# Wangshihu12/Voxel-SLAM

Hardware: AMD Instinct MI355X
Metric: local-BA iterations/sec (200k pts, W=10) (higher is better)
Workload: dtype f64

## Files before the change

### voxel-slam_amd/csrc/vba_kernels_factor.hpp

```cpp
#pragma once
#include <hip/hip_runtime.h>
#include "vba_eig3.hpp"

namespace vba {

struct FactorView {
  double *cl;
  double *fix;
  double *coe;
  double *eigval;
  double *eigvec;
  double *pcr;
  unsigned int *occ;
  int *tiles;
  int vs;
  int W;
};

__host__ __device__ inline int mask_bucket(unsigned int m, int nb) {
  constexpr int C[11][11] = {{1, 0, 0, 0, 0, 0, 0, 0, 0, 0, 0}, {1, 1, 0, 0, 0, 0, 0, 0, 0, 0, 0}, {1, 2, 1, 0, 0, 0, 0, 0, 0, 0, 0}, {1, 3, 3, 1, 0, 0, 0, 0, 0, 0, 0},
                             {1, 4, 6, 4, 1, 0, 0, 0, 0, 0, 0}, {1, 5, 10, 10, 5, 1, 0, 0, 0, 0, 0}, {1, 6, 15, 20, 15, 6, 1, 0, 0, 0, 0},
                             {1, 7, 21, 35, 35, 21, 7, 1, 0, 0, 0}, {1, 8, 28, 56, 70, 56, 28, 8, 1, 0, 0}, {1, 9, 36, 84, 126, 126, 84, 36, 9, 1, 0},
                             {1, 10, 45, 120, 210, 252, 210, 120, 45, 10, 1}};
  int p = 0;
// ... 344 lines not shown
  if (lane == 63) partial[blockIdx.x] = r;
  if (STAMPS && lane == 0 && blockIdx.x < 2048) {
    st3 = clock64();
    long long *o = stamps + (size_t)blockIdx.x * 4;
    o[0] = st0; o[1] = st1; o[2] = st2; o[3] = st3;
  }
}

__global__ __launch_bounds__(256) void k_reduce_partials(const double *__restrict__ partial, int nb, int nout, double *__restrict__ out,
                                                        const int *__restrict__ gate) {
  __shared__ double s[256];
  const int gate_v = gate ? *gate : 1;
  const int j = threadIdx.x & 15, q = threadIdx.x >> 4;
  const int o = blockIdx.x * 16 + j, oc = o < nout ? o : nout - 1;
  double pv[16];
#pragma unroll
  for (int k = 0; k < 16; k++) { const int b = q + 16 * k; pv[k] = partial[(size_t)(b < nb ? b : 0) * nout + oc]; }
#pragma unroll
  for (int k = 0; k < 16; k++) asm volatile("" : "+v"(pv[k]));
  if (gate_v == 0) return;
  double acc = 0.0;
  if (o < nout) {
#pragma unroll
    for (int k = 0; k < 16; k++) acc += (q + 16 * k < nb) ? pv[k] : 0.0;
    for (int b = q + 256; b < nb; b += 16) acc += partial[(size_t)b * nout + o];
  }
  s[threadIdx.x] = acc;
  __syncthreads();
  if (q == 0 && o < nout) {
    double t = 0.0;
#pragma unroll
    for (int k = 0; k < 16; k++) t += s[16 * k + j];
    out[o] = t;
  }
}

__global__ __launch_bounds__(256) void k_sum_scalar(const double *__restrict__ partial, int nb, double *__restrict__ out,
                                                   const int *__restrict__ gate) {
  __shared__ double s[4];
  if (gate && *gate == 0) return;
  double acc = 0.0;
  for (int b = threadIdx.x; b < nb; b += 256) acc += partial[b];
  acc = wave_sum(acc);
  if ((threadIdx.x & 63) == 0) s[threadIdx.x >> 6] = acc;
  __syncthreads();
  if (threadIdx.x == 0) out[0] = (s[0] + s[1]) + (s[2] + s[3]);
}

typedef double v4f64 __attribute__((ext_vector_type(4)));

constexpr int hess2_tv(int W) {
  return W == 2 ? 128 : W == 3 ? 80 : W == 4 ? 64 : W == 5 ? 48 : W == 6 ? 40 : (W == 7 || W == 8) ? 32 : (W == 9 || W == 10) ? 24 : 16;
}
constexpr int gcd_i(int a, int b) { return b == 0 ? a : gcd_i(b, a % b); }

__device__ __forceinline__ double rcp_f64(double x) {
  double y = __builtin_amdgcn_rcp(x);
  y = y * (2.0 - x * y);
  y = y * (2.0 - x * y);
  return y;
}

template <int W>
struct HessCfg2 {
  static constexpr int TV = hess2_tv(W);
  static constexpr int NT = 256;
  static constexpr int NC = 6 * W;
  static constexpr int NT16 = (NC + 15) / 16;
  static constexpr int NCP = 16 * NT16;
  static constexpr int GS = ((NCP % 32 == 16) ? NCP : NCP + 16) + 1;
  static constexpr int NK = 3 * TV;
  static constexpr int NWV = NT / 64;
  static constexpr int NU = NT16 * (NT16 + 1) / 2;
  static constexpr int KS = NWV / gcd_i(NU, NWV);
  static constexpr int UPW = NU * KS / NWV;
  static constexpr int KSTEPS = NK / 4 / KS;
  static constexpr int NOUT = NC * NC + NC + 1;
  static constexpr int EB = NU * 256;
  static constexpr int GB = EB + 21 * W;
  static constexpr int RB = GB + 6 * W;
  static constexpr int NOUT2 = RB + 1;
  static constexpr int NG8 = NT / 8;
  static_assert(TV * W <= NT && TV % 8 == 0 && (NK / 4) % KS == 0 && (NU * KS) % NWV == 0, "tile shape");
  static constexpr bool PRESCALE = ((size_t)2 * NK * GS + NK + W * 12 + 8) * sizeof(double) <= (size_t)150 * 1024;
  static constexpr size_t LDS_MAIN = (size_t)NK * GS * (PRESCALE ? 2 : 1) + NK + W * 12 + 8;
  static constexpr size_t LDS_EPI = (size_t)(KS > 1 ? NU * 256 : 0) + (size_t)28 * NG8 + 8;
  static constexpr size_t LDS_BYTES = (LDS_MAIN > LDS_EPI ? LDS_MAIN : LDS_EPI) * sizeof(double);
};

struct SlotLoad {
  double n, c[9], coe, l0, l1, l2, NN, vs0, vs1, vs2, U[9];
  bool valid;
};

template <int W>
__device__ __forceinline__ void slot_load(const FactorView &f, int v, int fi, int end, unsigned int occm, SlotLoad &q) {
  const size_t vs = (size_t)f.vs, fs = (size_t)W * vs;
  q.valid = v < end;
  if (q.valid) {
    const double *cp = f.cl + (size_t)fi * vs + v;
    const bool on = (occm >> fi) & 1u;
    q.n = on ? cp[9 * fs] : 0.0;
#pragma unroll
    for (int k = 0; k < 9; k++) q.c[k] = on ? cp[(size_t)k * fs] : 0.0;
    q.coe = f.coe[v];
    q.l0 = f.eigval[v]; q.l1 = f.eigval[vs + v]; q.l2 = f.eigval[2 * vs + v];
    q.NN = f.pcr[9 * vs + v]; q.vs0 = f.pcr[6 * vs + v]; q.vs1 = f.pcr[7 * vs + v]; q.vs2 = f.pcr[8 * vs + v];
#pragma unroll
    for (int k = 0; k < 9; k++) q.U[k] = f.eigvec[(size_t)k * vs + v];
  }
}

__device__ __forceinline__ void slot_terms(const SlotLoad &q, const double *R, bool first, double *g1, double *g2, double *hh, double &ck1, double &ck2, double &ck3,
                                           double *Err, double *Ert, double *Ett, double *gj, double &rres) {
if (q.valid) {
  const double coe = q.coe, l0 = q.l0, NN = q.NN;
  const double inn = rcp_f64(NN);
  const double c1 = 2.0 * rcp_f64(l0 - q.l1), c2 = 2.0 * rcp_f64(l0 - q.l2);
  ck1 = coe * c1; ck2 = coe * c2; ck3 = coe * (-2.0 * inn * inn);
  if (first) rres += coe * l0;
  const double n = q.n;
  if (n != 0.0) {
    const double pxx = q.c[0], pxy = q.c[1], pxz = q.c[2], pyy = q.c[3], pyz = q.c[4], pzz = q.c[5];
    const double vx = q.c[6], vy = q.c[7], vz = q.c[8];
    const double u00 = q.U[0], u01 = q.U[1], u02 = q.U[2], u10 = q.U[3], u11 = q.U[4], u12 = q.U[5], u20 = q.U[6], u21 = q.U[7], u22 = q.U[8];
    const double bx = q.vs0 * inn, by = q.vs1 * inn, bz = q.vs2 * inn;
    
    const double k0 = u00, k1 = u10, k2 = u20;
    const double a00 = R[0] * k0 + R[3] * k1 + R[6] * k2, a01 = R[1] * k0 + R[4] * k1 + R[7] * k2, a02 = R[2] * k0 + R[5] * k1 + R[8] * k2;
    const double a10 = R[0] * u01 + R[3] * u11 + R[6] * u21, a11 = R[1] * u01 + R[4] * u11 + R[7] * u21, a12 = R[2] * u01 + R[5] * u11 + R[8] * u21;
    const double a20 = R[0] * u02 + R[3] * u12 + R[6] * u22, a21 = R[1] * u02 + R[4] * u12 + R[7] * u22, a22 = R[2] * u02 + R[5] * u12 + R[8] * u22;
    const double tx = R[9] - bx, ty = R[10] - by, tz = R[11] - bz;
    const double s0 = k0 * tx + k1 * ty + k2 * tz, s1 = u01 * tx + u11 * ty + u21 * tz, s2 = u02 * tx + u12 * ty + u22 * tz;
    const double pa00 = pxx * a00 + pxy * a01 + pxz * a02, pa01 = pxy * a00 + pyy * a01 + pyz * a02, pa02 = pxz * a00 + pyz * a01 + pzz * a02;
    const double pa10 = pxx * a10 + pxy * a11 + pxz * a12, pa11 = pxy * a10 + pyy * a11 + pyz * a12, pa12 = pxz * a10 + pyz * a11 + pzz * a12;
    const double pa20 = pxx * a20 + pxy * a21 + pxz * a22, pa21 = pxy * a20 + pyy * a21 + pyz * a22, pa22 = pxz * a20 + pyz * a21 + pzz * a22;
    const double wx = pa00 + s0 * vx, wy = pa01 + s0 * vy, wz = pa02 + s0 * vz;
    const double c2x = R[0] * vx + R[1] * vy + R[2] * vz + n * tx;
    const double c2y = R[3] * vx + R[4] * vy + R[5] * vz + n * ty;
    const double c2z = R[6] * vx + R[7] * vy + R[8] * vz + n * tz;
    const double qx = vy * a02 - vz * a01, qy = vz * a00 - vx * a02, qz = vx * a01 - vy * a00;
    const double d0 = c2x * k0 + c2y * k1 + c2z * k2;
    const double d1 = c2x * u01 + c2y * u11 + c2z * u21;
    const double d2 = c2x * u02 + c2y * u12 + c2z * u22;
    const double j0 = 2.0 * (wy * a02 - wz * a01) * inn, j1 = 2.0 * (wz * a00 - wx * a02) * inn, j2 = 2.0 * (wx * a01 - wy * a00) * inn;
    const double j3 = 2.0 * d0 * k0 * inn, j4 = 2.0 * d0 * k1 * inn, j5 = 2.0 * d0 * k2 * inn;
    gj[0] += coe * j0; gj[1] += coe * j1; gj[2] += coe * j2; gj[3] += coe * j3; gj[4] += coe * j4; gj[5] += coe * j5;
    {
      const double bx1 = pa10 + s1 * vx, by1 = pa11 + s1 * vy, bz1 = pa12 + s1 * vz;
      g1[0] = (-(a01 * bz1 - a02 * by1) + (wy * a12 - wz * a11)) * inn;
      g1[1] = (-(a02 * bx1 - a00 * bz1) + (wz * a10 - wx * a12)) * inn;
      g1[2] = (-(a00 * by1 - a01 * bx1) + (wx * a11 - wy * a10)) * inn;
      g1[3] = (k0 * d1 + d0 * u01) * inn; g1[4] = (k1 * d1 + d0 * u11) * inn; g1[5] = (k2 * d1 + d0 * u21) * inn;
      const double bx2 = pa20 + s2 * vx, by2 = pa21 + s2 * vy, bz2 = pa22 + s2 * vz;
      g2[0] = (-(a01 * bz2 - a02 * by2) + (wy * a22 - wz * a21)) * inn;
      g2[1] = (-(a02 * bx2 - a00 * bz2) + (wz * a20 - wx * a22)) * inn;
      g2[2] = (-(a00 * by2 - a01 * bx2) + (wx * a21 - wy * a20)) * inn;
      g2[3] = (k0 * d2 + d0 * u02) * inn; g2[4] = (k1 * d2 + d0 * u12) * inn; g2[5] = (k2 * d2 + d0 * u22) * inn;
    }
    hh[0] = qx; hh[1] = qy; hh[2] = qz; hh[3] = n * k0; hh[4] = n * k1; hh[5] = n * k2;
    const double wa = wx * a00 + wy * a01 + wz * a02;
    const double t00 = a01 * pxz - a02 * pxy, t10 = a02 * pxx - a00 * pxz, t20 = a00 * pxy - a01 * pxx;
    const double t01 = a01 * pyz - a02 * pyy, t11 = a02 * pxy - a00 * pyz, t21 = a00 * pyy - a01 * pxy;
    const double t02 = a01 * pzz - a02 * pyz, t12 = a02 * pxz - a00 * pzz, t22 = a00 * pyz - a01 * pxz;
    const double S00 = t01 * a02 - t02 * a01, S01 = -t00 * a02 + t02 * a00, S02 = t00 * a01 - t01 * a00;
    const double S11 = -t10 * a02 + t12 * a00, S12 = t10 * a01 - t11 * a00;
    const double S22 = t20 * a01 - t21 * a00;
    const double e2 = 2.0 * inn * coe;
    Err[0] += e2 * (a00 * wx - wa - S00);
    Err[1] += e2 * (0.5 * (a00 * wy + wx * a01) - S01);
    Err[2] += e2 * (0.5 * (a00 * wz + wx * a02) - S02);
    Err[3] += e2 * (a01 * wy - wa - S11);
    Err[4] += e2 * (0.5 * (a01 * wz + wy * a02) - S12);
    Err[5] += e2 * (a02 * wz - wa - S22);
    Ert[0] += e2 * qx * k0; Ert[1] += e2 * qx * k1; Ert[2] += e2 * qx * k2;
    Ert[3] += e2 * qy * k0; Ert[4] += e2 * qy * k1; Ert[5] += e2 * qy * k2;
    Ert[6] += e2 * qz * k0; Ert[7] += e2 * qz * k1; Ert[8] += e2 * qz * k2;
    const double e3 = e2 * n;
    Ett[0] += e3 * k0 * k0; Ett[1] += e3 * k0 * k1; Ett[2] += e3 * k0 * k2; Ett[3] += e3 * k1 * k1; Ett[4] += e3 * k1 * k2; Ett[5] += e3 * k2 * k2;
  }
}
}

struct LmDev;
__device__ int lm_prev_stop(const LmDev *s);
__device__ double lm_r1(const LmDev *s);
__device__ const double *lm_xt(const LmDev *s);
__device__ void lm_update_apply(LmDev *s, double r2, int W);
__device__ __forceinline__ double lm_sum_partials(const double *__restrict__ r2_dev, int nb, int lane) {
  double pv[8];
#pragma unroll
  for (int k = 0; k < 8; k++) { const int b = lane + 64 * k; pv[k] = r2_dev[(nb > 0 && b < nb) ? b : 0]; }
  double acc = 0.0;
#pragma unroll
  for (int k = 0; k < 8; k++) acc += (lane + 64 * k < nb) ? pv[k] : 0.0;
  for (int b = lane + 512; b < nb; b += 64) acc += r2_dev[b];
  for (int m = 32; m >= 1; m >>= 1) acc += __shfl_xor(acc, m, 64);
  return acc;
}

struct LiDev;
struct LiJob { const LmDev *lm; LiDev *dev; const double *imu; double *himu, *gimu; };
__device__ void li_imu_body(const LmDev *s, LiDev *li, const double *imu, double *himu, double *gimu, double *lds);

template <int W>
__global__ __launch_bounds__(HessCfg2<W>::NT) void k_hessian2(FactorView f, const double *__restrict__ poses, int head, int end,
                                                             int ntiles, double *__restrict__ partial, const int *__restrict__ gate,
                                                             long long *__restrict__ stamps, LmDev *lm, const double *__restrict__ k4_partial, int k4_nb,
                                                             int nwg, LiJob li) {
  using C = HessCfg2<W>;
  extern __shared__ __attribute__((aligned(16))) double lds[];
  if (li.dev && blockIdx.x == 0) {
    li_imu_body(li.lm, li.dev, li.imu, li.himu, li.gimu, lds);
    return;
  }
  const int bid = (int)blockIdx.x - (li.dev ? 1 : 0);
  const int tile0 = (int)(((long long)bid * ntiles) / nwg), tile1 = (int)(((long long)(bid + 1) * ntiles) / nwg);
  const int my_vl = threadIdx.x % HessCfg2<W>::TV, my_fi = threadIdx.x / HessCfg2<W>::TV;
  unsigned int occ_nx = 0;
  if (my_fi < W && tile0 < tile1) { const int v0 = head + tile0 * HessCfg2<W>::TV + my_vl; occ_nx = f.occ[v0 < end ? v0 : end - 1]; }
  __shared__ int lm_dec[2];
  int gate_v = (gate && !lm) ? *gate : 1;
  double lm_r2 = 0.0;
  if (lm) {
    if (threadIdx.x < 64) {
      lm_r2 = lm_sum_partials(k4_partial, k4_nb, threadIdx.x);
      if (threadIdx.x == 0) {
        const double r1 = lm_r1(lm);
        const int stop = lm_prev_stop(lm);
        const bool accept = (r1 - lm_r2) > 0, nstop = fabs((r1 - lm_r2) / r1) < 1e-6;
        lm_dec[0] = (!stop && accept && !nstop) ? 1 : 0;
        lm_dec[1] = stop;
      }
    }
    poses = lm_xt(lm);
  }
#define VBA_STAMP(i) do { if (stamps && threadIdx.x == 0) stamps[(size_t)bid * 16 + (i)] = wall_clock64(); } while (0)
  VBA_STAMP(0);
  double *G = lds;
  double *GA = C::PRESCALE ? G + (size_t)C::NK * C::GS : G;
  double *cK = GA + (size_t)C::NK * C::GS;
  double *sp = cK + C::NK;
  const int tid = threadIdx.x, lane = tid & 63, wv = tid >> 6;

  for (int t = tid; t < W * 12; t += C::NT) sp[t] = poses[t];
  constexpr int PADC = C::GS - C::NC;
  if constexpr (PADC > 0)
    for (int t = tid; t < C::NK * PADC; t += C::NT) { G[(size_t)(t / PADC) * C::GS + C::NC + t % PADC] = 0.0; if (C::PRESCALE) GA[(size_t)(t / PADC) * C::GS + C::NC + t % PADC] = 0.0; }

  const int vl = tid % C::TV, fi = tid / C::TV;
  const bool slot_thread = fi < W;
  v4f64 acc[C::UPW];
#pragma unroll
  for (int t = 0; t < C::UPW; t++) acc[t] = (v4f64){0.0, 0.0, 0.0, 0.0};
  double Err[6] = {0, 0, 0, 0, 0, 0}, Ert[9] = {0, 0, 0, 0, 0, 0, 0, 0, 0}, Ett[6] = {0, 0, 0, 0, 0, 0};
  double gj[6] = {0, 0, 0, 0, 0, 0};
  double rres = 0.0;

  SlotLoad nx;
  nx.valid = false;
  if (slot_thread && tile0 < tile1) slot_load<W>(f, head + tile0 * C::TV + vl, fi, end, occ_nx, nx);
  if (slot_thread && tile0 + 1 < tile1) { const int v1 = head + (tile0 + 1) * C::TV + vl; occ_nx = f.occ[v1 < end ? v1 : end - 1]; }
  asm volatile("" : "+v"(nx.n));
  if (gate_v == 0) return;
  __syncthreads();
  if (lm) {
    const int run = lm_dec[0], was_stopped = lm_dec[1];
    if (bid == 0 && threadIdx.x < 64 && !was_stopped) lm_update_apply(lm, lm_r2, W);
    if (!run) return;
  }
  VBA_STAMP(1);
  int stamp_i = 2;

  for (int tile = tile0; tile < tile1; tile++) {
    if (slot_thread) {
      const SlotLoad q = nx;
      double g1[6] = {0, 0, 0, 0, 0, 0}, g2[6] = {0, 0, 0, 0, 0, 0}, hh[6] = {0, 0, 0, 0, 0, 0};
      double ck1 = 0.0, ck2 = 0.0, ck3 = 0.0;
      slot_terms(q, sp + 12 * fi, fi == 0, g1, g2, hh, ck1, ck2, ck3, Err, Ert, Ett, gj, rres);
      double *g = G + (size_t)(3 * vl) * C::GS + 6 * fi;
#pragma unroll
      for (int d = 0; d < 6; d++) { g[d] = g1[d]; g[C::GS + d] = g2[d]; g[2 * C::GS + d] = hh[d]; }
      if (C::PRESCALE) {
        double *ga = GA + (size_t)(3 * vl) * C::GS + 6 * fi;
#pragma unroll
        for (int d = 0; d < 6; d++) { ga[d] = g1[d] * ck1; ga[C::GS + d] = g2[d] * ck2; ga[2 * C::GS + d] = hh[d] * ck3; }
      }
      if (fi == 0) { cK[3 * vl] = ck1; cK[3 * vl + 1] = ck2; cK[3 * vl + 2] = ck3; }
      const int nt = tile + 1;
      nx.valid = false;
      if (nt < tile1) {
        slot_load<W>(f, head + nt * C::TV + vl, fi, end, occ_nx, nx);
        if (nt + 1 < tile1) { const int v2 = head + (nt + 1) * C::TV + vl; occ_nx = f.occ[v2 < end ? v2 : end - 1]; }
      }
    }
    __syncthreads();
    if (stamp_i < 12) { VBA_STAMP(stamp_i); stamp_i++; }
    {
      const int kr = lane >> 4, cl = lane & 15;
      const double *gap[C::UPW], *gbp[C::UPW], *ckp[C::UPW];
#pragma unroll
      for (int t = 0; t < C::UPW; t++) {
        const int unit = wv * C::UPW + t;
        const int u = unit % C::NU, ksp = unit / C::NU;
        int p = u, ta = 0;
        while (p >= C::NT16 - ta) { p -= C::NT16 - ta; ta++; }
        const int tb = ta + p;
        const int kb = ksp * C::KSTEPS * 4;
        gap[t] = GA + (size_t)(kb + kr) * C::GS + 16 * ta + cl;
        gbp[t] = G + (size_t)(kb + kr) * C::GS + 16 * tb + cl;
        ckp[t] = cK + kb + kr;
      }
      double ar[C::UPW], cr[C::UPW], br[C::UPW];
#pragma unroll
      for (int t = 0; t < C::UPW; t++) { ar[t] = gap[t][0]; cr[t] = C::PRESCALE ? 1.0 : ckp[t][0]; br[t] = gbp[t][0]; }
#pragma unroll
      for (int ks = 0; ks < C::KSTEPS; ks++) {
        double av[C::UPW], bv[C::UPW];
#pragma unroll
        for (int t = 0; t < C::UPW; t++) { av[t] = C::PRESCALE ? ar[t] : ar[t] * cr[t]; bv[t] = br[t]; }
        if (ks + 1 < C::KSTEPS) {
          const int k = 4 * (ks + 1);
#pragma unroll
          for (int t = 0; t < C::UPW; t++) { ar[t] = gap[t][(size_t)k * C::GS]; if (!C::PRESCALE) cr[t] = ckp[t][k]; br[t] = gbp[t][(size_t)k * C::GS]; }
        }
        __builtin_amdgcn_sched_barrier(0);
#pragma unroll
        for (int t = 0; t < C::UPW; t++) acc[t] = __builtin_amdgcn_mfma_f64_16x16x4f64(av[t], bv[t], acc[t], 0, 0, 0);
        __builtin_amdgcn_sched_barrier(0);
      }
    }
    __syncthreads();
    if (stamp_i < 12) { VBA_STAMP(stamp_i); stamp_i++; }
  }
  VBA_STAMP(12);

  double *out = partial + (size_t)bid * C::NOUT2;
  double *Tb = lds;
  double *Eb = Tb + (C::KS > 1 ? C::NU * 256 : 0);
  if (C::KS > 1) {
#pragma unroll
    for (int t = 0; t < C::UPW; t++) {
      const int unit = wv * C::UPW + t;
      if (unit / C::NU != 0) {
        const int u = unit % C::NU;
#pragma unroll
        for (int r = 0; r < 4; r++) {
          if (unit / C::NU == 1) Tb[u * 256 + r * 64 + lane] = acc[t][r];
        }
      }
    }
    for (int ksp = 2; ksp < C::KS; ksp++) {
      __syncthreads();
#pragma unroll
      for (int t = 0; t < C::UPW; t++) {
        const int unit = wv * C::UPW + t;
        if (unit / C::NU == ksp) {
          const int u = unit % C::NU;
#pragma unroll
          for (int r = 0; r < 4; r++) Tb[u * 256 + r * 64 + lane] += acc[t][r];
        }
      }
    }
  }
#pragma unroll
  for (int k = 0; k < 6; k++) { Err[k] = group8_sum(Err[k]); Ett[k] = group8_sum(Ett[k]); gj[k] = group8_sum(gj[k]); }
#pragma unroll
  for (int k = 0; k < 9; k++) Ert[k] = group8_sum(Ert[k]);
  rres = group8_sum(rres);
  if ((tid & 7) == 0) {
    const int g8 = tid >> 3;
#pragma unroll
    for (int k = 0; k < 6; k++) { Eb[(size_t)k * C::NG8 + g8] = Err[k]; Eb[(size_t)(15 + k) * C::NG8 + g8] = Ett[k]; Eb[(size_t)(21 + k) * C::NG8 + g8] = gj[k]; }
#pragma unroll
    for (int k = 0; k < 9; k++) Eb[(size_t)(6 + k) * C::NG8 + g8] = Ert[k];
    Eb[(size_t)27 * C::NG8 + g8] = rres;
  }
  __syncthreads();
  VBA_STAMP(13);
#pragma unroll
  for (int t = 0; t < C::UPW; t++) {
    const int unit = wv * C::UPW + t;
    if (unit / C::NU == 0) {
      const int u = unit % C::NU;
#pragma unroll
      for (int r = 0; r < 4; r++) {
        double val = acc[t][r];
        if (C::KS > 1) val += Tb[u * 256 + r * 64 + lane];
        out[u * 256 + r * 64 + lane] = val;
      }
    }
  }
  for (int t = tid; t < 28 * W; t += C::NT) {
    const int k = t % 28, fr = t / 28;
    double sum = 0.0;
#pragma unroll
    for (int g = 0; g < C::TV / 8; g++) sum += Eb[(size_t)k * C::NG8 + fr * (C::TV / 8) + g];
    if (k < 21) out[C::EB + 21 * fr + k] = sum;
    else if (k < 27) out[C::GB + 6 * fr + (k - 21)] = sum;
    else if (fr == 0) out[C::RB] = sum;
  }
  VBA_STAMP(14);
#undef VBA_STAMP
}

template <int W>
__device__ __forceinline__ double tl_fetch(const double *__restrict__ red, int row, int col) {
  using C = HessCfg2<W>;
  if (row > col) { const int t = row; row = col; col = t; }
  const int ta = row >> 4, tb = col >> 4;
  const int u = ta * C::NT16 - ta * (ta - 1) / 2 + (tb - ta);
  const int rt = row & 15, ct = col & 15;
  double val = red[u * 256 + (rt >> 2) * 64 + (rt & 3) * 16 + ct];
  const int fr = row / 6;
  if (col / 6 == fr) {
    const int a = row - 6 * fr, b = col - 6 * fr;
    int idx;
    if (b < 3) idx = a * 3 - a * (a - 1) / 2 + (b - a);
    else if (a < 3) idx = 6 + 3 * a + (b - 3);
    else { const int a2 = a - 3, b2 = b - 3; idx = 15 + a2 * 3 - a2 * (a2 - 1) / 2 + (b2 - a2); }
    val += red[C::EB + 21 * fr + idx];
  }
  return val;
}

template <int W>
__global__ void k_tiles_to_full(const double *__restrict__ red, double *__restrict__ full) {
  using C = HessCfg2<W>;
  for (int t = blockIdx.x * blockDim.x + threadIdx.x; t < C::NOUT; t += gridDim.x * blockDim.x) {
    if (t < C::NC * C::NC) full[t] = tl_fetch<W>(red, t / C::NC, t % C::NC);
    else if (t < C::NC * C::NC + C::NC) full[t] = red[C::GB + (t - C::NC * C::NC)];
    else full[t] = red[C::RB];
  }
}

}
```

### voxel-slam_amd/csrc/voxelba.hip

```cpp
#include "../../include/voxelba.h"

#define VBA_MAX_WIN_DEV VBA_MAX_WIN
#include "vba_kernels_factor.hpp"
#include "vba_kernels_h3.hpp"
#include "vba_kernels_map.hpp"
#include "vba_kernels_lm.hpp"
#include "vba_kernels_li.hpp"
#include "vba_kernels_scan.hpp"
#include "vba_kernels_gba.hpp"
#include "vba_kernels_big.hpp"
#include "vba_kernels_kd.hpp"
#include "vba_kernels_init.hpp"
#include "vba_kernels_btc.hpp"
#include "vba_io.hpp"
#include <cstddef>
#include "vba_hostmath.hpp"

#include <hip/hip_runtime.h>
#include <rccl/rccl.h>
#include <dlfcn.h>
#include <cstdio>
#include <cstdlib>
#include <cstring>
#include <atomic>
// ... 158 lines not shown
  hipEventCreate(&s.a); hipEventCreate(&s.b);
  hipEventRecord(s.a, c->stream);
}
void span_end(vba_ctx *c, const char *name, TimedSpan &s) {
  if (!s.a) return;
  hipEventRecord(s.b, c->stream);
  c->spans[name].push_back(s);
}

int ensure_pin(vba_ctx *c, size_t n) {
  if (n <= c->pin_doubles) return VBA_OK;
  if (c->h_pin) hipHostFree(c->h_pin);
  c->h_pin = nullptr; c->pin_doubles = 0;
  HIPCHK(c, hipHostMalloc((void **)&c->h_pin, n * sizeof(double), hipHostMallocDefault));
  c->pin_doubles = n;
  return VBA_OK;
}
int ensure_stage(vba_ctx *c, size_t bytes) {
  if (bytes <= c->stage_bytes) return VBA_OK;
  if (c->d_stage) hipFree(c->d_stage);
  c->d_stage = nullptr; c->stage_bytes = 0;
  HIPCHK(c, hipMalloc(&c->d_stage, bytes));
  c->stage_bytes = bytes;
  return VBA_OK;
}

int factor_reserve(vba_ctx *c, int need) {
  if (need <= c->cap) return VBA_OK;
  int newcap = c->cap ? c->cap : 4096;
  while (newcap < need) newcap *= 2;
  newcap = (newcap + 63) / 64 * 64 + 64 * 33;
  const int W = c->opt.win_size;
  FactorView n = c->fv;
  n.vs = newcap; n.W = W;
  const size_t rows[6] = {(size_t)10 * W, 10, 1, 3, 9, 10};
  double **np[6] = {&n.cl, &n.fix, &n.coe, &n.eigval, &n.eigvec, &n.pcr};
  double *op[6] = {c->fv.cl, c->fv.fix, c->fv.coe, c->fv.eigval, c->fv.eigvec, c->fv.pcr};
  for (int k = 0; k < 6; k++) {
    HIPCHK(c, hipMalloc((void **)np[k], rows[k] * newcap * sizeof(double)));
    HIPCHK(c, hipMemsetAsync(*np[k], 0, rows[k] * newcap * sizeof(double), c->stream));
    if (c->nvox > 0 && op[k])
      HIPCHK(c, hipMemcpy2DAsync(*np[k], (size_t)newcap * sizeof(double), op[k], (size_t)c->cap * sizeof(double),
                                 (size_t)c->nvox * sizeof(double), rows[k], hipMemcpyDeviceToDevice, c->stream));
  }
  unsigned int *oocc = c->fv.occ;
  int *otiles = c->fv.tiles;
  HIPCHK(c, hipMalloc((void **)&n.tiles, ((size_t)4 * newcap + 16) * sizeof(int)));
  HIPCHK(c, hipMemsetAsync(n.tiles, 0, ((size_t)4 * newcap + 16) * sizeof(int), c->stream));
  HIPCHK(c, hipMalloc((void **)&n.occ, (size_t)newcap * sizeof(unsigned int)));
  HIPCHK(c, hipMemsetAsync(n.occ, 0, (size_t)newcap * sizeof(unsigned int), c->stream));
  if (c->nvox > 0 && oocc) HIPCHK(c, hipMemcpyAsync(n.occ, oocc, (size_t)c->nvox * sizeof(unsigned int), hipMemcpyDeviceToDevice, c->stream));
  HIPCHK(c, hipStreamSynchronize(c->stream));
  for (int k = 0; k < 6; k++) if (op[k]) hipFree(op[k]);
  if (oocc) hipFree(oocc);
  if (otiles) hipFree(otiles);
  c->fv = n;
  if (c->nvox > 0 && c->use_h3) hipLaunchKernelGGL(k_factor_tiles, dim3(1), dim3(1024), 0, c->stream, c->fv, c->nvox);
  c->cap = newcap;
  return VBA_OK;
}

void factor_update_mask(vba_ctx *c, int base, int n) {
  if (n > 0) hipLaunchKernelGGL(k_factor_mask, dim3((n + 255) / 256), dim3(256), 0, c->stream, c->fv, base, n);
  if (base + n > 0 && c->use_h3) hipLaunchKernelGGL(k_factor_tiles, dim3(1), dim3(1024), 0, c->stream, c->fv, base + n);
}

int upload_poses(vba_ctx *c, const double *poses) {
  const int W = c->opt.win_size;
  int st = ensure_pin(c, 65536);
  if (st) return st;
  std::memcpy(c->h_pin, poses, (size_t)W * 12 * sizeof(double));
  HIPCHK(c, hipMemcpyAsync(c->d_poses, c->h_pin, (size_t)W * 12 * sizeof(double), hipMemcpyHostToDevice, c->stream));
  return VBA_OK;
}

template <int W>
int launch_hessian2_t(vba_ctx *c, const double *poses_dev, const int *gate, int head, int end, int *nblocks_out, LmDev *lm, const double *k4p, int k4nb,
                      const LiJob &li, size_t li_lds) {
  using C = HessCfg2<W>;
  const int ntiles = (end - head + C::TV - 1) / C::TV;
  const int maxb = li.dev ? c->max_blocks_hess - 1 : c->max_blocks_hess;
  int nb = ntiles < maxb ? ntiles : maxb;
  if (nb < 1) nb = 1;
  static bool attr_set[kMaxDevices] = {false};
  if (!attr_set[c->device % kMaxDevices]) {
    const size_t li_max = 150 * 1024;
    hipFuncSetAttribute((const void *)k_hessian2<W>, hipFuncAttributeMaxDynamicSharedMemorySize, (int)(C::LDS_BYTES > li_max ? C::LDS_BYTES : li_max));
    attr_set[c->device % kMaxDevices] = true;
  }
  long long *stamps = nullptr;
  static const bool want_stamps = diag_env("VBA_K3_STAMPS") != nullptr;
  if (want_stamps) {
    static long long *d_st = nullptr;
    if (!d_st) hipMalloc((void **)&d_st, (size_t)kMaxBlocksHess * 16 * 8);
    hipMemsetAsync(d_st, 0, (size_t)kMaxBlocksHess * 16 * 8, c->stream);
    stamps = d_st;
  }
  const size_t lds = (li.dev && li_lds > C::LDS_BYTES) ? li_lds : C::LDS_BYTES;
  hipLaunchKernelGGL(k_hessian2<W>, dim3(nb + (li.dev ? 1 : 0)), dim3(C::NT), lds, c->stream, c->fv, poses_dev, head, end, ntiles, c->d_partial, gate, stamps, lm, k4p, k4nb,
                     nb, li);
  if (want_stamps) {
    std::vector<long long> h((size_t)nb * 16);
    hipStreamSynchronize(c->stream);
    hipMemcpy(h.data(), stamps, h.size() * 8, hipMemcpyDeviceToHost);
    long long t0 = h[0];
    for (int b = 0; b < nb; b++) if (h[(size_t)b * 16] && h[(size_t)b * 16] < t0) t0 = h[(size_t)b * 16];
    for (int b : {0, 1, nb / 2, nb - 1}) {
      fprintf(stderr, "[k3 stamps] wg %d:", b);
      for (int i = 0; i < 15; i++) fprintf(stderr, " %lld", h[(size_t)b * 16 + i] ? h[(size_t)b * 16 + i] - t0 : -1);
      fprintf(stderr, "\n");
    }
    long long tmax = 0;
    for (int b = 0; b < nb; b++) if (h[(size_t)b * 16 + 14] - t0 > tmax) tmax = h[(size_t)b * 16 + 14] - t0;
    fprintf(stderr, "[k3 stamps] last workgroup ends at %lld ticks (100 MHz wall clock: 1 tick = 10 ns)\n", tmax);
  }
  *nblocks_out = nb;
  return VBA_OK;
}

template <int W>
int launch_hessian3_t(vba_ctx *c, const double *poses_dev, const int *gate, int *nblocks_out, LmDev *lm, const double *k4p, int k4nb, const LiJob &li, size_t li_lds) {
  using C = HessCfg3<W>;
  const int nb = li.dev ? c->max_blocks_hess - 1 : c->max_blocks_hess;
  static bool attr_set[kMaxDevices] = {false};
  if (!attr_set[c->device % kMaxDevices]) {
    const size_t li_max = 150 * 1024;
    hipFuncSetAttribute((const void *)k_hessian3<W>, hipFuncAttributeMaxDynamicSharedMemorySize, (int)(C::LDS_BYTES > li_max ? C::LDS_BYTES : li_max));
    attr_set[c->device % kMaxDevices] = true;
  }
  const size_t lds = (li.dev && li_lds > C::LDS_BYTES) ? li_lds : C::LDS_BYTES;
  long long *stamps = nullptr;
  static const bool want_stamps = diag_env("VBA_K3_STAMPS") != nullptr;
  if (want_stamps) {
    static long long *d_st = nullptr;
    if (!d_st) hipMalloc((void **)&d_st, (size_t)kMaxBlocksHess * 16 * 8);
    hipMemsetAsync(d_st, 0, (size_t)kMaxBlocksHess * 16 * 8, c->stream);
    stamps = d_st;
  }
  hipLaunchKernelGGL(k_hessian3<W>, dim3(nb + (li.dev ? 1 : 0)), dim3(C::NT), lds, c->stream, c->fv, poses_dev, c->nvox, c->d_partial, gate, lm, k4p, k4nb, nb, li, stamps);
  if (want_stamps) {
    std::vector<long long> h((size_t)nb * 16);
    hipStreamSynchronize(c->stream);
    hipMemcpy(h.data(), stamps, h.size() * 8, hipMemcpyDeviceToHost);
    long long t0 = h[0];
    for (int b = 0; b < nb; b++) if (h[(size_t)b * 16] && h[(size_t)b * 16] < t0) t0 = h[(size_t)b * 16];
    for (int b : {0, 1, nb / 2, nb - 1}) {
      fprintf(stderr, "[k3 stamps] wg %d:", b);
      for (int i = 0; i < 16; i++) fprintf(stderr, " %lld", h[(size_t)b * 16 + i] ? h[(size_t)b * 16 + i] - t0 : -1);
      fprintf(stderr, "\n");
    }
    long long tmax = 0;
    for (int b = 0; b < nb; b++) if (h[(size_t)b * 16 + 15] - t0 > tmax) tmax = h[(size_t)b * 16 + 15] - t0;
    fprintf(stderr, "[k3 stamps] last workgroup ends at %lld ticks (100 MHz wall clock: 1 tick = 10 ns); per workgroup: start, prologue, then per tile [A, B, combine, E]\n", tmax);
  }
  *nblocks_out = nb;
  return VBA_OK;
}

int launch_hessian(vba_ctx *c, const double *pd, const int *gate, int head, int end, int *nb, LmDev *lm = nullptr, const double *k4p = nullptr, int k4nb = 0,
                   const LiJob &li = LiJob{}, size_t li_lds = 0) {
  if (head == 0 && end == c->nvox && c->opt.win_size <= 10 && c->use_h3) {
    switch (c->opt.win_size) {
#define VBA_H3_CASE(WW) case WW: return launch_hessian3_t<WW>(c, pd, gate, nb, lm, k4p, k4nb, li, li_lds);
      VBA_H3_CASE(2) VBA_H3_CASE(3) VBA_H3_CASE(4) VBA_H3_CASE(5) VBA_H3_CASE(6) VBA_H3_CASE(7) VBA_H3_CASE(8) VBA_H3_CASE(9) VBA_H3_CASE(10)
#undef VBA_H3_CASE
    }
  }
  switch (c->opt.win_size) {
#define VBA_H_CASE(WW) case WW: return launch_hessian2_t<WW>(c, pd, gate, head, end, nb, lm, k4p, k4nb, li, li_lds);
    VBA_H_CASE(2) VBA_H_CASE(3) VBA_H_CASE(4) VBA_H_CASE(5) VBA_H_CASE(6) VBA_H_CASE(7) VBA_H_CASE(8) VBA_H_CASE(9) VBA_H_CASE(10)
    VBA_H_CASE(11) VBA_H_CASE(12) VBA_H_CASE(13) VBA_H_CASE(14) VBA_H_CASE(15) VBA_H_CASE(16)
#undef VBA_H_CASE
    default: return VBA_ERR_UNSUPPORTED_WINDOW;
  }
}

#ifndef VBA_K4_TV
#define VBA_K4_TV 32
#endif
inline bool residual_vpl(const vba_ctx *c, int n) { return n > c->residual_vpl_from; }
inline int residual_nb(const vba_ctx *c, int n) { return residual_vpl(c, n) ? (n + 63) / 64 : (n + VBA_K4_TV - 1) / VBA_K4_TV; }

void k4_stamps_dump(vba_ctx *c, int nb, long long *d_st) {
// ... 2630 lines not shown
```

Before: 21660.

## Run two ping-pong Hessian pipelines per workgroup and fold scaling into sqrt

Splits the Hessian kernel into a non-LI variant for W<=10 that runs two half-workgroups, each with its own LDS image. They are staggered by one phase, so one half builds the slot Jacobians while the other runs the MFMA accumulation. The per-row coefficient weighting is folded into both operands through sqrt(-ck), and the result is negated on output. This drops the separate prescaled copy and cK buffer. The cost is doubled threads and LDS per block, and relying on ck being non-positive for sqrt to be exact.

```diff
diff --git a/voxel-slam_amd/csrc/vba_kernels_factor.hpp b/voxel-slam_amd/csrc/vba_kernels_factor.hpp
--- a/voxel-slam_amd/csrc/vba_kernels_factor.hpp
+++ b/voxel-slam_amd/csrc/vba_kernels_factor.hpp
@@ -450,10 +450,18 @@
   static constexpr int NOUT2 = RB + 1;
   static constexpr int NG8 = NT / 8;
   static_assert(TV * W <= NT && TV % 8 == 0 && (NK / 4) % KS == 0 && (NU * KS) % NWV == 0, "tile shape");
-  static constexpr bool PRESCALE = ((size_t)2 * NK * GS + NK + W * 12 + 8) * sizeof(double) <= (size_t)150 * 1024;
-  static constexpr size_t LDS_MAIN = (size_t)NK * GS * (PRESCALE ? 2 : 1) + NK + W * 12 + 8;
-  static constexpr size_t LDS_EPI = (size_t)(KS > 1 ? NU * 256 : 0) + (size_t)28 * NG8 + 8;
+};
+
+template <int W, bool LI>
+struct HessShape2 {
+  using C = HessCfg2<W>;
+  static constexpr size_t IMG = (size_t)C::NK * C::GS;
+  static constexpr int NH = (!LI && W <= 10 && (2 * IMG + W * 12 + 8) * sizeof(double) <= (size_t)160 * 1024) ? 2 : 1;
+  static constexpr int NT = C::NT * NH;
+  static constexpr size_t LDS_MAIN = NH * IMG + W * 12 + 8;
+  static constexpr size_t LDS_EPI = (size_t)(NH * C::KS - 1) * C::NU * 256 + (size_t)28 * C::NG8 * NH + 8;
   static constexpr size_t LDS_BYTES = (LDS_MAIN > LDS_EPI ? LDS_MAIN : LDS_EPI) * sizeof(double);
+  static_assert(NH == 1 || LDS_BYTES <= (size_t)160 * 1024, "two pipelines must fit a CU's LDS");
 };
 
 struct SlotLoad {
@@ -571,22 +579,32 @@
 struct LiJob { const LmDev *lm; LiDev *dev; const double *imu; double *himu, *gimu; };
 __device__ void li_imu_body(const LmDev *s, LiDev *li, const double *imu, double *himu, double *gimu, double *lds);
 
-template <int W>
-__global__ __launch_bounds__(HessCfg2<W>::NT) void k_hessian2(FactorView f, const double *__restrict__ poses, int head, int end,
-                                                             int ntiles, double *__restrict__ partial, const int *__restrict__ gate,
-                                                             long long *__restrict__ stamps, LmDev *lm, const double *__restrict__ k4_partial, int k4_nb,
-                                                             int nwg, LiJob li) {
+template <int W, bool LI>
+__global__ __launch_bounds__((HessShape2<W, LI>::NT)) void k_hessian2(FactorView f, const double *__restrict__ poses, int head, int end,
+                                                                     int ntiles, double *__restrict__ partial, const int *__restrict__ gate,
+                                                                     long long *__restrict__ stamps, LmDev *lm, const double *__restrict__ k4_partial, int k4_nb,
+                                                                     int nwg, LiJob li) {
   using C = HessCfg2<W>;
+  using L = HessShape2<W, LI>;
+  constexpr int NH = L::NH;
   extern __shared__ __attribute__((aligned(16))) double lds[];
-  if (li.dev && blockIdx.x == 0) {
-    li_imu_body(li.lm, li.dev, li.imu, li.himu, li.gimu, lds);
-    return;
-  }
-  const int bid = (int)blockIdx.x - (li.dev ? 1 : 0);
+  if constexpr (LI) {
+    if (li.dev && blockIdx.x == 0) {
+      li_imu_body(li.lm, li.dev, li.imu, li.himu, li.gimu, lds);
+      return;
+    }
+  }
+  const int bid = (int)blockIdx.x - ((LI && li.dev) ? 1 : 0);
+  const int tid = threadIdx.x, lane = tid & 63;
+  const int wv = __builtin_amdgcn_readfirstlane(tid >> 6);
+  const int hf = wv / C::NWV, hw = wv % C::NWV, ht = tid - hf * C::NT;
   const int tile0 = (int)(((long long)bid * ntiles) / nwg), tile1 = (int)(((long long)(bid + 1) * ntiles) / nwg);
-  const int my_vl = threadIdx.x % HessCfg2<W>::TV, my_fi = threadIdx.x / HessCfg2<W>::TV;
+  const int ntl = tile1 - tile0;
+  const int cnt = (ntl - hf + NH - 1) / NH;
+  const int vl = ht % C::TV, fi = ht / C::TV;
+  const bool slot_thread = fi < W;
   unsigned int occ_nx = 0;
-  if (my_fi < W && tile0 < tile1) { const int v0 = head + tile0 * HessCfg2<W>::TV + my_vl; occ_nx = f.occ[v0 < end ? v0 : end - 1]; }
+  if (slot_thread && cnt > 0) { const int v0 = head + (tile0 + hf) * C::TV + vl; occ_nx = f.occ[v0 < end ? v0 : end - 1]; }
   __shared__ int lm_dec[2];
   int gate_v = (gate && !lm) ? *gate : 1;
   double lm_r2 = 0.0;
@@ -605,19 +623,14 @@
   }
 #define VBA_STAMP(i) do { if (stamps && threadIdx.x == 0) stamps[(size_t)bid * 16 + (i)] = wall_clock64(); } while (0)
   VBA_STAMP(0);
-  double *G = lds;
-  double *GA = C::PRESCALE ? G + (size_t)C::NK * C::GS : G;
-  double *cK = GA + (size_t)C::NK * C::GS;
-  double *sp = cK + C::NK;
-  const int tid = threadIdx.x, lane = tid & 63, wv = tid >> 6;
-
-  for (int t = tid; t < W * 12; t += C::NT) sp[t] = poses[t];
+  double *G = lds + hf * L::IMG;
+  double *sp = lds + NH * L::IMG;
+
+  for (int t = tid; t < W * 12; t += L::NT) sp[t] = poses[t];
   constexpr int PADC = C::GS - C::NC;
   if constexpr (PADC > 0)
-    for (int t = tid; t < C::NK * PADC; t += C::NT) { G[(size_t)(t / PADC) * C::GS + C::NC + t % PADC] = 0.0; if (C::PRESCALE) GA[(size_t)(t / PADC) * C::GS + C::NC + t % PADC] = 0.0; }
-
-  const int vl = tid % C::TV, fi = tid / C::TV;
-  const bool slot_thread = fi < W;
+    for (int t = tid; t < NH * C::NK * PADC; t += L::NT) lds[(size_t)(t / PADC) * C::GS + C::NC + t % PADC] = 0.0;
+
   v4f64 acc[C::UPW];
 #pragma unroll
   for (int t = 0; t < C::UPW; t++) acc[t] = (v4f64){0.0, 0.0, 0.0, 0.0};
@@ -627,8 +640,8 @@
 
   SlotLoad nx;
   nx.valid = false;
-  if (slot_thread && tile0 < tile1) slot_load<W>(f, head + tile0 * C::TV + vl, fi, end, occ_nx, nx);
-  if (slot_thread && tile0 + 1 < tile1) { const int v1 = head + (tile0 + 1) * C::TV + vl; occ_nx = f.occ[v1 < end ? v1 : end - 1]; }
+  if (slot_thread && cnt > 0) slot_load<W>(f, head + (tile0 + hf) * C::TV + vl, fi, end, occ_nx, nx);
+  if (slot_thread && cnt > 1) { const int v1 = head + (tile0 + hf + NH) * C::TV + vl; occ_nx = f.occ[v1 < end ? v1 : end - 1]; }
   asm volatile("" : "+v"(nx.n));
   if (gate_v == 0) return;
   __syncthreads();
@@ -640,95 +653,96 @@
   VBA_STAMP(1);
   int stamp_i = 2;
 
-  for (int tile = tile0; tile < tile1; tile++) {
+  auto phase_a = [&](int i) {
     if (slot_thread) {
       const SlotLoad q = nx;
       double g1[6] = {0, 0, 0, 0, 0, 0}, g2[6] = {0, 0, 0, 0, 0, 0}, hh[6] = {0, 0, 0, 0, 0, 0};
       double ck1 = 0.0, ck2 = 0.0, ck3 = 0.0;
       slot_terms(q, sp + 12 * fi, fi == 0, g1, g2, hh, ck1, ck2, ck3, Err, Ert, Ett, gj, rres);
+      const double s1 = __builtin_sqrt(0.0 - ck1), s2 = __builtin_sqrt(0.0 - ck2), s3 = __builtin_sqrt(0.0 - ck3);
       double *g = G + (size_t)(3 * vl) * C::GS + 6 * fi;
 #pragma unroll
-      for (int d = 0; d < 6; d++) { g[d] = g1[d]; g[C::GS + d] = g2[d]; g[2 * C::GS + d] = hh[d]; }
-      if (C::PRESCALE) {
-        double *ga = GA + (size_t)(3 * vl) * C::GS + 6 * fi;
-#pragma unroll
-        for (int d = 0; d < 6; d++) { ga[d] = g1[d] * ck1; ga[C::GS + d] = g2[d] * ck2; ga[2 * C::GS + d] = hh[d] * ck3; }
+      for (int d = 0; d < 6; d++) { g[d] = g1[d] * s1; g[C::GS + d] = g2[d] * s2; g[2 * C::GS + d] = hh[d] * s3; }
+      const int nt = tile0 + hf + NH * (i + 1);
+      nx.valid = false;
+      if (i + 1 < cnt) {
+        slot_load<W>(f, head + nt * C::TV + vl, fi, end, occ_nx, nx);
+        if (i + 2 < cnt) { const int v2 = head + (nt + NH) * C::TV + vl; occ_nx = f.occ[v2 < end ? v2 : end - 1]; }
       }
-      if (fi == 0) { cK[3 * vl] = ck1; cK[3 * vl + 1] = ck2; cK[3 * vl + 2] = ck3; }
-      const int nt = tile + 1;
-      nx.valid = false;
-      if (nt < tile1) {
-        slot_load<W>(f, head + nt * C::TV + vl, fi, end, occ_nx, nx);
-        if (nt + 1 < tile1) { const int v2 = head + (nt + 1) * C::TV + vl; occ_nx = f.occ[v2 < end ? v2 : end - 1]; }
+    }
+  };
+  auto phase_b = [&]() {
+    const double *Gl = G + (size_t)(lane >> 4) * C::GS + (lane & 15);
+    int oa[C::UPW], ob[C::UPW];
+    const double *pa[C::UPW], *pb[C::UPW];
+#pragma unroll
+    for (int t = 0; t < C::UPW; t++) {
+      const int unit = hw * C::UPW + t;
+      const int u = unit % C::NU, ksp = unit / C::NU;
+      int pu = u, ta = 0;
+      while (pu >= C::NT16 - ta) { pu -= C::NT16 - ta; ta++; }
+      const int tb = ta + pu;
+      const int kb = ksp * C::KSTEPS * 4;
+      oa[t] = kb * C::GS + 16 * ta;
+      ob[t] = kb * C::GS + 16 * tb;
+      pa[t] = Gl + oa[t];
+      pb[t] = Gl + ob[t];
+    }
+    double ar[C::UPW], br[C::UPW];
+#pragma unroll
+    for (int t = 0; t < C::UPW; t++) { ar[t] = NH == 2 ? Gl[oa[t]] : pa[t][0]; br[t] = NH == 2 ? Gl[ob[t]] : pb[t][0]; }
+#pragma unroll
+    for (int ks = 0; ks < C::KSTEPS; ks++) {
+      double av[C::UPW], bv[C::UPW];
+#pragma unroll
+      for (int t = 0; t < C::UPW; t++) { av[t] = ar[t]; bv[t] = br[t]; }
+      if (ks + 1 < C::KSTEPS) {
+        const int k = 4 * (ks + 1) * C::GS;
+#pragma unroll
+        for (int t = 0; t < C::UPW; t++) { ar[t] = NH == 2 ? Gl[oa[t] + k] : pa[t][k]; br[t] = NH == 2 ? Gl[ob[t] + k] : pb[t][k]; }
       }
-    }
-    __syncthreads();
-    if (stamp_i < 12) { VBA_STAMP(stamp_i); stamp_i++; }
-    {
-      const int kr = lane >> 4, cl = lane & 15;
-      const double *gap[C::UPW], *gbp[C::UPW], *ckp[C::UPW];
-#pragma unroll
-      for (int t = 0; t < C::UPW; t++) {
-        const int unit = wv * C::UPW + t;
-        const int u = unit % C::NU, ksp = unit / C::NU;
-        int p = u, ta = 0;
-        while (p >= C::NT16 - ta) { p -= C::NT16 - ta; ta++; }
-        const int tb = ta + p;
-        const int kb = ksp * C::KSTEPS * 4;
-        gap[t] = GA + (size_t)(kb + kr) * C::GS + 16 * ta + cl;
-        gbp[t] = G + (size_t)(kb + kr) * C::GS + 16 * tb + cl;
-        ckp[t] = cK + kb + kr;
+      __builtin_amdgcn_sched_barrier(0);
+#pragma unroll
+      for (int t = 0; t < C::UPW; t++) acc[t] = __builtin_amdgcn_mfma_f64_16x16x4f64(av[t], bv[t], acc[t], 0, 0, 0);
+      __builtin_amdgcn_sched_barrier(0);
+    }
+  };
+  if constexpr (NH == 1) {
+    for (int i = 0; i < ntl; i++) {
+      phase_a(i);
+      __syncthreads();
+      if (stamp_i < 12) { VBA_STAMP(stamp_i); stamp_i++; }
+      phase_b();
+      __syncthreads();
+      if (stamp_i < 12) { VBA_STAMP(stamp_i); stamp_i++; }
+    }
+  } else {
+    const int cnt0 = (ntl + 1) / 2, cnt1 = ntl / 2;
+    const int nsteps = 2 * cnt0 > 2 * cnt1 + 1 ? 2 * cnt0 : 2 * cnt1 + 1;
+    for (int s = 0; s < nsteps; s++) {
+      const int p = s - hf, i = p >> 1;
+      if (p >= 0 && i < cnt) {
+        if ((p & 1) == 0) phase_a(i);
+        else phase_b();
       }
-      double ar[C::UPW], cr[C::UPW], br[C::UPW];
-#pragma unroll
-      for (int t = 0; t < C::UPW; t++) { ar[t] = gap[t][0]; cr[t] = C::PRESCALE ? 1.0 : ckp[t][0]; br[t] = gbp[t][0]; }
-#pragma unroll
-      for (int ks = 0; ks < C::KSTEPS; ks++) {
-        double av[C::UPW], bv[C::UPW];
-#pragma unroll
-        for (int t = 0; t < C::UPW; t++) { av[t] = C::PRESCALE ? ar[t] : ar[t] * cr[t]; bv[t] = br[t]; }
-        if (ks + 1 < C::KSTEPS) {
-          const int k = 4 * (ks + 1);
-#pragma unroll
-          for (int t = 0; t < C::UPW; t++) { ar[t] = gap[t][(size_t)k * C::GS]; if (!C::PRESCALE) cr[t] = ckp[t][k]; br[t] = gbp[t][(size_t)k * C::GS]; }
-        }
-        __builtin_amdgcn_sched_barrier(0);
-#pragma unroll
-        for (int t = 0; t < C::UPW; t++) acc[t] = __builtin_amdgcn_mfma_f64_16x16x4f64(av[t], bv[t], acc[t], 0, 0, 0);
-        __builtin_amdgcn_sched_barrier(0);
-      }
-    }
-    __syncthreads();
-    if (stamp_i < 12) { VBA_STAMP(stamp_i); stamp_i++; }
+      __syncthreads();
+      if (stamp_i < 12) { VBA_STAMP(stamp_i); stamp_i++; }
+    }
   }
   VBA_STAMP(12);
 
+  constexpr int NPART = NH * C::KS;
   double *out = partial + (size_t)bid * C::NOUT2;
   double *Tb = lds;
-  double *Eb = Tb + (C::KS > 1 ? C::NU * 256 : 0);
-  if (C::KS > 1) {
-#pragma unroll
-    for (int t = 0; t < C::UPW; t++) {
-      const int unit = wv * C::UPW + t;
-      if (unit / C::NU != 0) {
-        const int u = unit % C::NU;
-#pragma unroll
-        for (int r = 0; r < 4; r++) {
-          if (unit / C::NU == 1) Tb[u * 256 + r * 64 + lane] = acc[t][r];
-        }
-      }
-    }
-    for (int ksp = 2; ksp < C::KS; ksp++) {
-      __syncthreads();
-#pragma unroll
-      for (int t = 0; t < C::UPW; t++) {
-        const int unit = wv * C::UPW + t;
-        if (unit / C::NU == ksp) {
-          const int u = unit % C::NU;
-#pragma unroll
-          for (int r = 0; r < 4; r++) Tb[u * 256 + r * 64 + lane] += acc[t][r];
-        }
-      }
+  double *Eb = Tb + (size_t)(NPART - 1) * C::NU * 256;
+  constexpr int NGE = NH * C::NG8;
+#pragma unroll
+  for (int t = 0; t < C::UPW; t++) {
+    const int unit = hw * C::UPW + t;
+    const int u = unit % C::NU, part = hf * C::KS + unit / C::NU;
+    if (part != 0) {
+#pragma unroll
+      for (int r = 0; r < 4; r++) Tb[(size_t)(part - 1) * C::NU * 256 + u * 256 + r * 64 + lane] = acc[t][r];
     }
   }
 #pragma unroll
@@ -739,31 +753,36 @@
   if ((tid & 7) == 0) {
     const int g8 = tid >> 3;
 #pragma unroll
-    for (int k = 0; k < 6; k++) { Eb[(size_t)k * C::NG8 + g8] = Err[k]; Eb[(size_t)(15 + k) * C::NG8 + g8] = Ett[k]; Eb[(size_t)(21 + k) * C::NG8 + g8] = gj[k]; }
-#pragma unroll
-    for (int k = 0; k < 9; k++) Eb[(size_t)(6 + k) * C::NG8 + g8] = Ert[k];
-    Eb[(size_t)27 * C::NG8 + g8] = rres;
+    for (int k = 0; k < 6; k++) { Eb[(size_t)k * NGE + g8] = Err[k]; Eb[(size_t)(15 + k) * NGE + g8] = Ett[k]; Eb[(size_t)(21 + k) * NGE + g8] = gj[k]; }
+#pragma unroll
+    for (int k = 0; k < 9; k++) Eb[(size_t)(6 + k) * NGE + g8] = Ert[k];
+    Eb[(size_t)27 * NGE + g8] = rres;
   }
   __syncthreads();
   VBA_STAMP(13);
-#pragma unroll
-  for (int t = 0; t < C::UPW; t++) {
-    const int unit = wv * C::UPW + t;
-    if (unit / C::NU == 0) {
-      const int u = unit % C::NU;
-#pragma unroll
-      for (int r = 0; r < 4; r++) {
-        double val = acc[t][r];
-        if (C::KS > 1) val += Tb[u * 256 + r * 64 + lane];
-        out[u * 256 + r * 64 + lane] = val;
+  if (hf == 0) {
+#pragma unroll
+    for (int t = 0; t < C::UPW; t++) {
+      const int unit = hw * C::UPW + t;
+      if (unit / C::NU == 0) {
+        const int u = unit % C::NU;
+#pragma unroll
+        for (int r = 0; r < 4; r++) {
+          double val = acc[t][r];
+#pragma unroll
+          for (int pt = 1; pt < NPART; pt++) val += Tb[(size_t)(pt - 1) * C::NU * 256 + u * 256 + r * 64 + lane];
+          out[u * 256 + r * 64 + lane] = -val;
+        }
       }
     }
   }
-  for (int t = tid; t < 28 * W; t += C::NT) {
+  for (int t = tid; t < 28 * W; t += L::NT) {
     const int k = t % 28, fr = t / 28;
     double sum = 0.0;
 #pragma unroll
-    for (int g = 0; g < C::TV / 8; g++) sum += Eb[(size_t)k * C::NG8 + fr * (C::TV / 8) + g];
+    for (int h = 0; h < NH; h++)
+#pragma unroll
+      for (int g = 0; g < C::TV / 8; g++) sum += Eb[(size_t)k * NGE + h * C::NG8 + fr * (C::TV / 8) + g];
     if (k < 21) out[C::EB + 21 * fr + k] = sum;
     else if (k < 27) out[C::GB + 6 * fr + (k - 21)] = sum;
     else if (fr == 0) out[C::RB] = sum;
diff --git a/voxel-slam_amd/csrc/voxelba.hip b/voxel-slam_amd/csrc/voxelba.hip
--- a/voxel-slam_amd/csrc/voxelba.hip
+++ b/voxel-slam_amd/csrc/voxelba.hip
@@ -264,10 +264,14 @@
   const int maxb = li.dev ? c->max_blocks_hess - 1 : c->max_blocks_hess;
   int nb = ntiles < maxb ? ntiles : maxb;
   if (nb < 1) nb = 1;
+  constexpr bool OWN = W <= 10;
+  using LL = HessShape2<W, !OWN>;
+  using LI = HessShape2<W, true>;
   static bool attr_set[kMaxDevices] = {false};
   if (!attr_set[c->device % kMaxDevices]) {
     const size_t li_max = 150 * 1024;
-    hipFuncSetAttribute((const void *)k_hessian2<W>, hipFuncAttributeMaxDynamicSharedMemorySize, (int)(C::LDS_BYTES > li_max ? C::LDS_BYTES : li_max));
+    if constexpr (OWN) hipFuncSetAttribute((const void *)k_hessian2<W, false>, hipFuncAttributeMaxDynamicSharedMemorySize, (int)LL::LDS_BYTES);
+    hipFuncSetAttribute((const void *)k_hessian2<W, true>, hipFuncAttributeMaxDynamicSharedMemorySize, (int)(LI::LDS_BYTES > li_max ? LI::LDS_BYTES : li_max));
     attr_set[c->device % kMaxDevices] = true;
   }
   long long *stamps = nullptr;
@@ -278,9 +282,14 @@
     hipMemsetAsync(d_st, 0, (size_t)kMaxBlocksHess * 16 * 8, c->stream);
     stamps = d_st;
   }
-  const size_t lds = (li.dev && li_lds > C::LDS_BYTES) ? li_lds : C::LDS_BYTES;
-  hipLaunchKernelGGL(k_hessian2<W>, dim3(nb + (li.dev ? 1 : 0)), dim3(C::NT), lds, c->stream, c->fv, poses_dev, head, end, ntiles, c->d_partial, gate, stamps, lm, k4p, k4nb,
-                     nb, li);
+  if (li.dev) {
+    const size_t lds = li_lds > LI::LDS_BYTES ? li_lds : LI::LDS_BYTES;
+    hipLaunchKernelGGL((k_hessian2<W, true>), dim3(nb + 1), dim3(LI::NT), lds, c->stream, c->fv, poses_dev, head, end, ntiles, c->d_partial, gate, stamps, lm,
+                       k4p, k4nb, nb, li);
+  } else {
+    hipLaunchKernelGGL((k_hessian2<W, !OWN>), dim3(nb), dim3(LL::NT), LL::LDS_BYTES, c->stream, c->fv, poses_dev, head, end, ntiles, c->d_partial, gate, stamps,
+                       lm, k4p, k4nb, nb, li);
+  }
   if (want_stamps) {
     std::vector<long long> h((size_t)nb * 16);
     hipStreamSynchronize(c->stream);
```

After: 21850, median of 6. No clear change (+0.9%).
